# sacs-epfl/decentralized-learning-simulator

Hardware: AMD Instinct MI355X
Metric: device-resident GB/s, N-way weighted model-tensor reduce; 1/2/4/8 MI355X (higher is better)
Workload: dtype f32

## Files before the change

decentralized-learning-simulator_amd/csrc/dispatch.hpp:

```cpp
#pragma once

#include <hip/hip_runtime.h>

#include <algorithm>
#include <cmath>
#include <cstdint>
#include <cstdlib>
#include <cstring>
#include <type_traits>
#include <vector>

#include "dlsim.h"
#include "wreduce_kernels.hpp"
#include "chunk_mean_kernels.hpp"
#include "ab_env.hpp"


namespace dlsim_host __attribute__((visibility("hidden"))) {

int fail(int code, const char* fmt, ...) __attribute__((format(printf, 2, 3)));
int hip_fail(hipError_t e, const char* what);

constexpr int kVpt = 4;
constexpr size_t kBatchSmallBytes = size_t{1} << 20;
// ... 10 lines not shown
constexpr size_t kMaxLaunchOutBytes = (size_t{1} << 31) - (size_t{1} << 20);
template <class Op> constexpr int max_fixed_fan_in() { return Op::kBytes >= 4 ? 14 : 9; }
template <class Op> constexpr int group_size() { return Op::kBytes >= 4 ? 8 : 4; }

struct Shape {
  int vpt;
  int store;
  bool wave;
};
template <class Op, int C> constexpr Shape fixed_shape() {
  if constexpr (Op::kBytes >= 4) {
    if constexpr (C == 0) return Shape{2, kStore, false};
    else if constexpr (C == 1) return Shape{4, kStore, false};
    else return Shape{4, kStore, true};
  } else {
    if constexpr (C < 2) return Shape{1, kStore, true};
    else return Shape{4, dlsim::kStNT, false};
  }
}
int device_cus();
inline bool v4_tiles_even(size_t nvec) {
  const double x = static_cast<double>(nvec / (static_cast<size_t>(dlsim::kBlock) * 4)) /
                   static_cast<double>(device_cus());
  return x >= 0.75 && std::ceil(x) / x <= 1.25;
}
inline bool small_shape_r04() {
  static const bool on = dlsim::ab_getenv("DLSIM_SMALL_SHAPE_R04") != nullptr;
  return on;
}
template <class Op> int size_class(size_t nelem, int fixed_fan_in = 0) {
  const size_t bytes = nelem * Op::kBytes;
  if constexpr (Op::kBytes >= 4) {
    if (bytes < 8000000)
      return Op::kBytes == 4 && fixed_fan_in >= 6 && !small_shape_r04() && v4_tiles_even(nelem / Op::E) ? 1 : 0;
    return bytes < 20000000 ? 1 : 2;
  } else {
    return bytes < 96000000 ? 0 : 2;
  }
}

inline bool aligned16(const void* p) { return (reinterpret_cast<uintptr_t>(p) & 15u) == 0; }

template <class S> inline const void* pre_ptr(const S& s, int nf, int i) { return i < nf ? s.p[i] : nullptr; }
static_assert(dlsim::kPre == 5, "the launches below pass five leading pointers");

template <class Op, class S, int NF, int VPT, int STP, bool WAVE>
hipError_t launch_shape(const S& s, int n, void* out, size_t nelem, hipStream_t st) {
  const size_t nvec = nelem / Op::E;
  const size_t tile = static_cast<size_t>(dlsim::kBlock) * VPT;
  const size_t blocks = nvec / tile + 1;
  if (blocks > 0x7fffffffu) return hipErrorInvalidValue;
  hipLaunchKernelGGL((dlsim::k_wreduce_tiles<Op, S, NF, group_size<Op>(), VPT, kNT, STP, WAVE>),
                     dim3(static_cast<unsigned>(blocks)), dim3(dlsim::kBlock), 0, st, s, n, out, nvec, nelem);
  return hipGetLastError();
}

template <class Op, int C> constexpr Shape grouped_shape() {
  if constexpr (C == 0) return Shape{1, kStore, true};
  else if constexpr (Op::kBytes >= 4) return Shape{4, kStore, false};
  else return Shape{4, dlsim::kStNT, false};
}

template <class Op, class S, int NF, int C>
hipError_t launch_class(const S& s, int n, void* out, size_t nelem, hipStream_t st) {
  constexpr Shape k = NF > 0 ? fixed_shape<Op, C>() : grouped_shape<Op, C>();
  return launch_shape<Op, S, NF, k.vpt, k.store, k.wave>(s, n, out, nelem, st);
}

constexpr int kDeferU = 2, kDeferRMin = 4, kDeferOneRoundMax = 24;
template <class Op, int NF> constexpr int defer_rmax() { return NF >= 12 ? 24 : 32; }
template <class Op, int NF> constexpr bool defer_eligible() { return Op::kBytes == 4 && (NF >= 2 || NF == 0); }
inline int defer_min_fan_in() {
  static const int k = [] {
    const char* e = dlsim::ab_getenv("DLSIM_DEFER_MIN_FAN_IN");
    return e ? std::atoi(e) : 3;
  }();
  return k;
}
constexpr int kDeferWideFanIn = 10;
constexpr size_t kDeferWideRowsPerCu = 16;
inline bool defer_on() {
  static const bool on = [] {
    const char* e = dlsim::ab_getenv("DLSIM_DEFER");
    return !(e && e[0] == '0');
  }();
  return on;
}
inline int defer_max_fan_in() {
  static const int k = [] {
    const char* e = dlsim::ab_getenv("DLSIM_DEFER_MAX_FAN_IN");
    return e ? std::atoi(e) : 1 << 30;
  }();
  return k;
}
inline int defer_r_override() {
  static const int r = [] {
    const char* e = dlsim::ab_getenv("DLSIM_DEFER_R");
    return e ? std::atoi(e) : 0;
  }();
  return r;
}
inline int defer_rows(size_t nvec, size_t cus, int rmax) {
  if (defer_r_override() > 0) return std::min(defer_r_override(), rmax);
  const size_t T = (nvec + dlsim::kDeferBlock - 1) / dlsim::kDeferBlock;
  const size_t one = ((T + cus - 1) / cus + 1) & ~size_t{1};
  if (one <= static_cast<size_t>(std::min(rmax, kDeferOneRoundMax))) return std::max(static_cast<int>(one), kDeferRMin);
  const size_t two = ((T + 2 * cus - 1) / (2 * cus) + 1) & ~size_t{1};
  if (two <= static_cast<size_t>(rmax)) return static_cast<int>(two);
  int best = rmax;
  double best_cost = 1e300;
  for (int R = rmax / 2; R <= rmax; R += 2) {
    const double w = static_cast<double>((T + R - 1) / R) / static_cast<double>(cus);
    const double full = std::floor(w), x = w - full;
    const double cost = R * (full + (x > 0 ? std::max(x, 0.38 + 0.45 * x) : 0.0)) + 0.1 * std::ceil(w);
    if (cost < best_cost - 1e-9) {
      best_cost = cost;
      best = R;
    }
  }
  return best;
}

inline bool defer_grouped_on() {
  static const bool on = [] {
    const char* e = dlsim::ab_getenv("DLSIM_DEFER_GROUPED");
    return !(e && e[0] == '0');
  }();
  return on;
}
constexpr double kDeferMinMB = 10.0;
inline double defer_min_mb() {
  static const double x = [] {
    const char* e = dlsim::ab_getenv("DLSIM_DEFER_MIN_MB");
    return e ? std::atof(e) : kDeferMinMB;
  }();
  return x;
}
template <class Op> bool use_defer(int n, size_t nelem) {
  if (Op::kBytes != 4 || n < std::max(2, defer_min_fan_in()) || n > defer_max_fan_in() || !defer_on()) return false;
  if (static_cast<double>(nelem * Op::kBytes) < defer_min_mb() * 1e6) return false;
  if (n > max_fixed_fan_in<Op>()) return defer_grouped_on();
  if (n <= kDeferWideFanIn) return true;
  const size_t rows = nelem / Op::E / dlsim::kDeferBlock;
  return rows >= kDeferWideRowsPerCu * static_cast<size_t>(device_cus());
}

template <class Op> const char* kernel_name(int n, size_t nelem) {
  if (nelem == 0 || n < 1) return "";
  const size_t first = std::min(nelem, kMaxLaunchOutBytes / Op::kBytes);
  if (use_defer<Op>(n, first)) return n <= max_fixed_fan_in<Op>() ? "dlsim::k_wreduce_defer_pre" : "dlsim::k_wreduce_defer";
  return "dlsim::k_wreduce_tiles";
}

template <class Op, class S, int NF, int RC>
hipError_t launch_defer_kernel(const S& s, int n, void* out, size_t nvec, size_t nelem, int R, unsigned blocks,
                               hipStream_t st) {
  if constexpr (NF > 0) {
    hipLaunchKernelGGL(
        (dlsim::k_wreduce_defer_pre<Op, S, NF, group_size<Op>(), defer_rmax<Op, NF>(), kDeferU, kStore, RC>),
        dim3(blocks), dim3(dlsim::kDeferBlock), 0, st, nvec, out, pre_ptr(s, NF, 0), pre_ptr(s, NF, 1),
        pre_ptr(s, NF, 2), pre_ptr(s, NF, 3), pre_ptr(s, NF, 4), s, n, R, nelem);
  } else {
    hipLaunchKernelGGL(
        (dlsim::k_wreduce_defer<Op, S, NF, group_size<Op>(), defer_rmax<Op, NF>(), kDeferU, kStore, RC>),
        dim3(blocks), dim3(dlsim::kDeferBlock), 0, st, s, n, R, out, nvec, nelem);
  }
  return hipGetLastError();
}

template <class Op, class S, int NF, int RC>
hipError_t launch_defer_rc(const S& s, int n, void* out, size_t nvec, size_t nelem, int R, unsigned blocks,
                           hipStream_t st) {
  if constexpr (RC > defer_rmax<Op, NF>()) {
    return launch_defer_kernel<Op, S, NF, 0>(s, n, out, nvec, nelem, R, blocks, st);
  } else {
    if (R == RC) return launch_defer_kernel<Op, S, NF, RC>(s, n, out, nvec, nelem, R, blocks, st);
    return launch_defer_rc<Op, S, NF, RC + kDeferU>(s, n, out, nvec, nelem, R, blocks, st);
  }
}

template <class Op, class S, int NF>
hipError_t launch_defer(const S& s, int n, void* out, size_t nelem, hipStream_t st) {
  const size_t nvec = nelem / Op::E;
  const int R = defer_rows(nvec, static_cast<size_t>(device_cus()), defer_rmax<Op, NF>());
  const size_t span = static_cast<size_t>(dlsim::kDeferBlock) * static_cast<size_t>(R);
  const size_t blocks = (nvec + span - 1) / span;
  if (blocks == 0 || blocks > 0x7fffffffu) return hipErrorInvalidValue;
  if constexpr (NF >= 3 && std::is_same<Op, dlsim::F32Exact>::value)
    return launch_defer_rc<Op, S, NF, kDeferRMin>(s, n, out, nvec, nelem, R, static_cast<unsigned>(blocks), st);
  return launch_defer_kernel<Op, S, NF, 0>(s, n, out, nvec, nelem, R, static_cast<unsigned>(blocks), st);
}

template <class Op, class S, int NF>
hipError_t launch_tiles(const S& s, int n, void* out, size_t nelem, hipStream_t st) {
  if constexpr (NF > 0) {
    const int c = size_class<Op>(nelem, NF);
    if constexpr (defer_eligible<Op, NF>())
      if (use_defer<Op>(NF, nelem)) return launch_defer<Op, S, NF>(s, n, out, nelem, st);
    switch (c) {
      case 0: return launch_class<Op, S, NF, 0>(s, n, out, nelem, st);
      case 1: return launch_class<Op, S, NF, 1>(s, n, out, nelem, st);
      default: return launch_class<Op, S, NF, 2>(s, n, out, nelem, st);
    }
  } else {
    if constexpr (defer_eligible<Op, 0>())
      if (use_defer<Op>(n, nelem)) return launch_defer<Op, S, 0>(s, n, out, nelem, st);
    return size_class<Op>(nelem) == 0 ? launch_class<Op, S, 0, 0>(s, n, out, nelem, st)
                                      : launch_class<Op, S, 0, 2>(s, n, out, nelem, st);
  }
}

template <class Op, int K>
hipError_t launch_fixed_k(const dlsim::Slots<16, dlsim::wt_t<Op>>& s, int n, void* out, size_t nelem,
                          hipStream_t st) {
  if constexpr (K > max_fixed_fan_in<Op>()) {
    return hipErrorInvalidValue;
  } else {
    if (n == K) return launch_tiles<Op, dlsim::Slots<16, dlsim::wt_t<Op>>, K>(s, n, out, nelem, st);
    return launch_fixed_k<Op, K + 1>(s, n, out, nelem, st);
  }
}

template <class Op, class S>
hipError_t launch_any(const S& s, int n, void* out, size_t nelem, bool vec, hipStream_t st) {
  if (vec) {
    if constexpr (std::is_same<S, dlsim::Slots<16, dlsim::wt_t<Op>>>::value) {
      if (n <= max_fixed_fan_in<Op>()) return launch_fixed_k<Op, 1>(s, n, out, nelem, st);
    }
    return launch_tiles<Op, S, 0>(s, n, out, nelem, st);
  }
  const size_t blocks = (nelem + dlsim::kBlock - 1) / dlsim::kBlock;
  if (blocks > 0x7fffffffu) return hipErrorInvalidValue;
  hipLaunchKernelGGL((dlsim::k_wreduce_scalar<Op, S>), dim3(static_cast<unsigned>(blocks)), dim3(dlsim::kBlock), 0,
                     st, s, n, out, nelem);
  return hipGetLastError();
}

template <int NB, class W>
void fill_slots(dlsim::Slots<NB, W>& s, const void* const* in, const W* w, int n, float div) {
  std::memset(&s, 0, sizeof(s));
  for (int i = 0; i < n; ++i) {
    s.p[i] = in[i];
    s.w[i] = w ? w[i] : 1.0f;
  }
  s.div = div;
}

template <class Op>
int run_range(const void* const* in, int n, const dlsim::wt_t<Op>* w, void* out, size_t nelem, bool vec, float div,
              hipStream_t st) {
  using W = dlsim::wt_t<Op>;
  hipError_t e;
  if (n <= 16) {
    dlsim::Slots<16, W> s;
    fill_slots(s, in, w, n, div);
    e = launch_any<Op>(s, n, out, nelem, vec, st);
  } else if (n <= DLSIM_MAX_FUSED_INPUTS) {
    dlsim::Slots<DLSIM_MAX_FUSED_INPUTS, W> s;
    fill_slots(s, in, w, n, div);
    e = launch_any<Op>(s, n, out, nelem, vec, st);
  } else {
    const size_t pbytes = static_cast<size_t>(n) * sizeof(void*);
    std::vector<unsigned char> h(pbytes + static_cast<size_t>(n) * sizeof(W));
    std::memcpy(h.data(), in, pbytes);
    for (int i = 0; i < n; ++i) {
      const W wi = w ? w[i] : W(1);
      std::memcpy(h.data() + pbytes + static_cast<size_t>(i) * sizeof(W), &wi, sizeof(W));
    }
    void* d = nullptr;
    e = hipMallocAsync(&d, h.size(), st);
    if (e != hipSuccess) return hip_fail(e, "fan-in table alloc");
    e = hipMemcpyAsync(d, h.data(), h.size(), hipMemcpyHostToDevice, st);
    if (e == hipSuccess) {
      const dlsim::DevSlots<W> s{static_cast<const void* const*>(d),
                                 reinterpret_cast<const W*>(static_cast<unsigned char*>(d) + pbytes), div};
      e = launch_any<Op>(s, n, out, nelem, vec, st);
    }
    const hipError_t e2 = hipFreeAsync(d, st);
    if (e == hipSuccess) e = e2;
  }
  if (e != hipSuccess) return hip_fail(e, "kernel launch");
  return DLSIM_OK;
}

template <class Op>
int run(const void* const* in, int n, const dlsim::wt_t<Op>* w, void* out, size_t nelem, hipStream_t st,
        float div = 1.0f) {
  if (nelem == 0) return DLSIM_OK;
  bool vec = aligned16(out);
  for (int i = 0; i < n && vec; ++i) vec = aligned16(in[i]);
  const size_t chunk = kMaxLaunchOutBytes / Op::kBytes;
  if (!vec || nelem <= chunk) return run_range<Op>(in, n, w, out, nelem, vec, div, st);
  std::vector<const void*> sub(static_cast<size_t>(n));
  for (size_t b = 0; b < nelem; b += chunk) {
    const size_t len = std::min(chunk, nelem - b);
    for (int i = 0; i < n; ++i) sub[i] = static_cast<const char*>(in[i]) + b * Op::kBytes;
    int rc = run_range<Op>(sub.data(), n, w, static_cast<char*>(out) + b * Op::kBytes, len, vec, div, st);
    if (rc != DLSIM_OK) return rc;
  }
  return DLSIM_OK;
}

struct Span {
  uintptr_t a, b;
  int task;
};

inline bool cross_task_overlap(int nt, const int* fan_in, const void* const* in, void* const* outs, const size_t* nelem,
                        size_t esz) {
  std::vector<Span> wr;
  wr.reserve(static_cast<size_t>(nt));
  for (int t = 0; t < nt; ++t) {
    if (nelem[t] == 0) continue;
    const uintptr_t a = reinterpret_cast<uintptr_t>(outs[t]);
// ... 558 lines not shown
```

decentralized-learning-simulator_amd/csrc/wreduce_kernels.hpp:

```cpp
#pragma once

#include <hip/hip_runtime.h>
#include <stdint.h>

#include <type_traits>

#pragma clang fp contract(off)

namespace dlsim {

constexpr int kBlock = 256;

typedef uint32_t u32x4 __attribute__((ext_vector_type(4)));
typedef float f32x2 __attribute__((ext_vector_type(2)));
typedef __bf16 bf16x2 __attribute__((ext_vector_type(2)));

__device__ __forceinline__ float bf16_round(float f) {
  uint32_t u = __float_as_uint(f);
  if ((u & 0x7fffffffu) > 0x7f800000u) return __uint_as_float(0x7fc00000u);
  u += 0x7fffu + ((u >> 16) & 1u);
  return __uint_as_float(u & 0xffff0000u);
}

__device__ __forceinline__ void bf16_round2(float& a0, float& a1) {
// ... 203 lines not shown
  using T = double;
  using W = double;
  static constexpr int E = 2;
  static constexpr int kBytes = 8;
  static constexpr int kFmt = kFmtF32;
  __device__ static double init(double) { return 0.0; }
  __device__ static double step(double acc, double, double x) { return acc + x; }
  __device__ static void step2(double& a0, double& a1, double, double x0, double x1) {
    a0 = a0 + x0;
    a1 = a1 + x1;
  }
  __device__ static double finish(double a, float div) { return a / static_cast<double>(div); }
};

template <class Op>
__device__ __forceinline__ void unpack(const u32x4& r, acc_t<Op> (&x)[Op::E]) {
  if constexpr (Op::kBytes == 8) {
#pragma unroll
    for (int e = 0; e < 2; ++e)
      x[e] = __builtin_bit_cast(double, static_cast<uint64_t>(r[2 * e]) | (static_cast<uint64_t>(r[2 * e + 1]) << 32));
  } else if constexpr (Op::kBytes == 4) {
#pragma unroll
    for (int e = 0; e < 4; ++e) x[e] = __uint_as_float(r[e]);
  } else if constexpr (Op::kFmt == kFmtF16) {
#pragma unroll
    for (int e = 0; e < 4; ++e) {
      const uint32_t u = r[e];
      x[2 * e] = static_cast<float>(__builtin_bit_cast(_Float16, static_cast<uint16_t>(u & 0xffffu)));
      x[2 * e + 1] = static_cast<float>(__builtin_bit_cast(_Float16, static_cast<uint16_t>(u >> 16)));
    }
  } else {
#pragma unroll
    for (int e = 0; e < 4; ++e) {
      x[2 * e] = __uint_as_float(r[e] << 16);
      x[2 * e + 1] = __uint_as_float(r[e] & 0xffff0000u);
    }
  }
}

template <class Op>
__device__ __forceinline__ u32x4 pack(const acc_t<Op> (&a)[Op::E], float div) {
  u32x4 r;
  if constexpr (Op::kBytes == 8) {
#pragma unroll
    for (int e = 0; e < 2; ++e) {
      const uint64_t u = __builtin_bit_cast(uint64_t, Op::finish(a[e], div));
      r[2 * e] = static_cast<uint32_t>(u);
      r[2 * e + 1] = static_cast<uint32_t>(u >> 32);
    }
  } else if constexpr (Op::kBytes == 4) {
#pragma unroll
    for (int e = 0; e < 4; ++e) r[e] = __float_as_uint(Op::finish(a[e], div));
  } else if constexpr (Op::kFmt == kFmtF16) {
#pragma unroll
    for (int e = 0; e < 4; ++e) {
      const uint32_t lo = __builtin_bit_cast(uint16_t, static_cast<_Float16>(Op::finish(a[2 * e], div)));
      const uint32_t hi = __builtin_bit_cast(uint16_t, static_cast<_Float16>(Op::finish(a[2 * e + 1], div)));
      r[e] = lo | (hi << 16);
    }
  } else {
#pragma unroll
    for (int e = 0; e < 4; ++e) {
      const uint32_t lo = __float_as_uint(Op::finish(a[2 * e], div)) >> 16;
      const uint32_t hi = __float_as_uint(Op::finish(a[2 * e + 1], div)) & 0xffff0000u;
      r[e] = lo | hi;
    }
  }
  return r;
}

template <class Op>
__device__ __forceinline__ acc_t<Op> load_elem(const void* p, size_t j) {
  if constexpr (Op::kBytes == 8) {
    return static_cast<const double*>(p)[j];
  } else if constexpr (Op::kBytes == 4) {
    return static_cast<const float*>(p)[j];
  } else if constexpr (Op::kFmt == kFmtF16) {
    return static_cast<float>(static_cast<const _Float16*>(p)[j]);
  } else {
    return __uint_as_float(static_cast<uint32_t>(static_cast<const uint16_t*>(p)[j]) << 16);
  }
}

template <class Op>
__device__ __forceinline__ void store_elem(void* p, size_t j, acc_t<Op> a, float div) {
  if constexpr (Op::kBytes == 8) {
    static_cast<double*>(p)[j] = Op::finish(a, div);
  } else if constexpr (Op::kBytes == 4) {
    static_cast<float*>(p)[j] = Op::finish(a, div);
  } else if constexpr (Op::kFmt == kFmtF16) {
    static_cast<_Float16*>(p)[j] = static_cast<_Float16>(Op::finish(a, div));
  } else {
    static_cast<uint16_t*>(p)[j] = static_cast<uint16_t>(__float_as_uint(Op::finish(a, div)) >> 16);
  }
}

constexpr int kLdBuffer = 100;

template <int LDP>
__device__ __forceinline__ u32x4 ld16(const void* base, size_t v) {
  if constexpr (LDP >= kLdBuffer) {
    const __amdgpu_buffer_rsrc_t r =
        __builtin_amdgcn_make_buffer_rsrc(const_cast<void*>(base), 0, 0x7fffffff, 0x00020000);
    return __builtin_bit_cast(u32x4, __builtin_amdgcn_raw_buffer_load_b128(r, static_cast<int>(v * 16), 0,
                                                                           LDP - kLdBuffer));
  } else {
    const u32x4* p = static_cast<const u32x4*>(base) + v;
    if constexpr (LDP == 1) return __builtin_nontemporal_load(p);
    else return *p;
  }
}

template <bool NT>
__device__ __forceinline__ void st16(void* base, size_t v, const u32x4& r) {
  u32x4* p = static_cast<u32x4*>(base) + v;
  if constexpr (NT) __builtin_nontemporal_store(r, p);
  else *p = r;
}

constexpr int kStPlain = -1;
constexpr int kStNT = -2;

struct OutRef {
  void* ptr;
  __amdgpu_buffer_rsrc_t rsrc;
};

template <int STP>
__device__ __forceinline__ void store_vec(const OutRef& o, size_t v, const u32x4& r) {
  if constexpr (STP == kStPlain) {
    st16<false>(o.ptr, v, r);
  } else if constexpr (STP == kStNT) {
    st16<true>(o.ptr, v, r);
  } else {
    __builtin_amdgcn_raw_buffer_store_b128(r, o.rsrc, static_cast<int>(v * 16), 0, STP);
  }
}

template <int STP>
__device__ __forceinline__ OutRef make_out(void* out, size_t nvec) {
  OutRef o;
  o.ptr = out;
  if constexpr (STP >= 0) {
    o.rsrc = __builtin_amdgcn_make_buffer_rsrc(out, 0, static_cast<int>(nvec * 16), 0x00020000);
  }
  return o;
}

template <int NB, class W = float>
struct Slots {
  const void* p[NB];
  W w[NB];
  float div;
  __device__ const void* ptr(int i) const { return p[i]; }
  __device__ W wt(int i) const { return w[i]; }
  __device__ float divisor() const { return div; }
};

template <class W = float>
struct DevSlots {
  const void* const* p;
  const W* w;
  float div;
  __device__ const void* ptr(int i) const { return p[i]; }
  __device__ W wt(int i) const { return w[i]; }
  __device__ float divisor() const { return div; }
};

template <class Op, class S>
__device__ __forceinline__ void fold_scalar(const S& s, int n, void* out, size_t j) {
  acc_t<Op> a = 0;
  for (int i = 0; i < n; i += 8) {
    acc_t<Op> x[8];
#pragma unroll
    for (int g = 0; g < 8; ++g) x[g] = (i + g < n) ? load_elem<Op>(s.ptr(i + g), j) : 0.0f;
    if (i == 0) a = Op::init(x[0]);
#pragma unroll
    for (int g = 0; g < 8; ++g)
      if (i + g < n) a = Op::step(a, s.wt(i + g), x[g]);
  }
  store_elem<Op>(out, j, a, s.divisor());
}

template <class Op, class S>
__global__ __launch_bounds__(kBlock) void k_wreduce_scalar(const S s, int n, void* __restrict__ out,
                                                           size_t nelem) {
  const size_t j = static_cast<size_t>(blockIdx.x) * kBlock + threadIdx.x;
  if (j < nelem) fold_scalar<Op, S>(s, n, out, j);
}

template <class Op, int VPT, int NT, bool CHECK, int VS = kBlock>
__device__ __forceinline__ void load_tile(const void* src, size_t v0, size_t nvec,
                                          u32x4 (&r)[VPT]) {
#pragma unroll
  for (int v = 0; v < VPT; ++v) {
    const size_t idx = v0 + static_cast<size_t>(v) * VS;
    if constexpr (CHECK) {
      r[v] = u32x4{0u, 0u, 0u, 0u};
      if (idx < nvec) r[v] = ld16<NT>(src, idx);
    } else {
      r[v] = ld16<NT>(src, idx);
    }
  }
}

template <class Op, int VPT>
__device__ __forceinline__ void fold_tile(acc_t<Op> (&a)[VPT][Op::E], wt_t<Op> w, const u32x4 (&r)[VPT]) {
#pragma unroll
  for (int v = 0; v < VPT; ++v) {
    acc_t<Op> x[Op::E];
    unpack<Op>(r[v], x);
#pragma unroll
    for (int e = 0; e < Op::E; e += 2) Op::step2(a[v][e], a[v][e + 1], w, x[e], x[e + 1]);
  }
}

template <class Op, int VPT>
__device__ __forceinline__ void init_tile(acc_t<Op> (&a)[VPT][Op::E], const u32x4 (&r)[VPT], bool from_acc) {
#pragma unroll
  for (int v = 0; v < VPT; ++v) {
    acc_t<Op> x[Op::E];
    unpack<Op>(r[v], x);
#pragma unroll
    for (int e = 0; e < Op::E; ++e) a[v][e] = from_acc ? x[e] : Op::init(x[e]);
  }
}

template <class Op, class S, int NF, int G, int VPT, int NT, bool CHECK, int STP, int VS = kBlock>
__device__ __forceinline__ void reduce_tile(const S& s, int n, const OutRef& out, size_t v0, size_t nvec) {
  acc_t<Op> a[VPT][Op::E];
  if constexpr (NF > 0) {
    u32x4 r[NF][VPT];
#pragma unroll
    for (int i = 0; i < NF; ++i) load_tile<Op, VPT, NT, CHECK, VS>(s.ptr(i), v0, nvec, r[i]);
    init_tile<Op, VPT>(a, r[0], false);
#pragma unroll
    for (int i = 0; i < NF; ++i) fold_tile<Op, VPT>(a, s.wt(i), r[i]);
  } else {
    {
      u32x4 r[G][VPT];
      const int cnt = n < G ? n : G;
#pragma unroll
      for (int g = 0; g < G; ++g)
        if (g < cnt) load_tile<Op, VPT, NT, CHECK, VS>(s.ptr(g), v0, nvec, r[g]);
      init_tile<Op, VPT>(a, r[0], false);
#pragma unroll
      for (int g = 0; g < G; ++g)
        if (g < cnt) fold_tile<Op, VPT>(a, s.wt(g), r[g]);
    }
    for (int i0 = G; i0 < n; i0 += G) {
      u32x4 r[G][VPT];
      const int cnt = (n - i0) < G ? (n - i0) : G;
#pragma unroll
      for (int g = 0; g < G; ++g)
        if (g < cnt) load_tile<Op, VPT, NT, CHECK, VS>(s.ptr(i0 + g), v0, nvec, r[g]);
#pragma unroll
      for (int g = 0; g < G; ++g)
        if (g < cnt) fold_tile<Op, VPT>(a, s.wt(i0 + g), r[g]);
    }
  }
#pragma unroll
  for (int v = 0; v < VPT; ++v) {
    const size_t idx = v0 + static_cast<size_t>(v) * VS;
    if (!CHECK || idx < nvec) store_vec<STP>(out, idx, pack<Op>(a[v], s.divisor()));
  }
}

template <class Op, class S, int NF, int G, int VPT, int NT, int STP, bool WAVEMAP>
__device__ __forceinline__ void tiles_body(const S& s, int n, void* __restrict__ out, size_t nvec, size_t nelem) {
  constexpr size_t kTile = static_cast<size_t>(kBlock) * VPT;
  const size_t full = nvec / kTile;
  const OutRef o = make_out<STP>(out, nvec);
  const size_t nb = gridDim.x;
  if (blockIdx.x == 0) {
    if (full * kTile < nvec)
      reduce_tile<Op, S, NF, G, VPT, NT, true, STP>(s, n, o, full * kTile + threadIdx.x, nvec);
    const size_t j = nvec * Op::E + threadIdx.x;
    if (j < nelem) fold_scalar<Op, S>(s, n, out, j);
    if (nb > 1) return;
  }
  const size_t workers = nb > 1 ? nb - 1 : 1;
  const size_t first = nb > 1 ? blockIdx.x - 1 : 0;
  if constexpr (WAVEMAP) {
    const size_t lane_off = (threadIdx.x >> 6) * 64 * VPT + (threadIdx.x & 63);
    for (size_t t = first; t < full; t += workers)
      reduce_tile<Op, S, NF, G, VPT, NT, false, STP, 64>(s, n, o, t * kTile + lane_off, nvec);
  } else {
    for (size_t t = first; t < full; t += workers)
      reduce_tile<Op, S, NF, G, VPT, NT, false, STP>(s, n, o, t * kTile + threadIdx.x, nvec);
  }
}

template <class Op, class S, int NF, int G, int VPT, int NT, int STP = (NT ? kStNT : kStPlain),
          bool WAVEMAP = false>
__global__ __launch_bounds__(kBlock) void k_wreduce_tiles(const S s, int n, void* __restrict__ out, size_t nvec,
                                                          size_t nelem) {
  tiles_body<Op, S, NF, G, VPT, NT, STP, WAVEMAP>(s, n, out, nvec, nelem);
}

constexpr int kPre = 5;
template <class S>
struct PreSlots {
  const void* q[kPre];
  const S& s;
  __device__ const void* ptr(int i) const { return i < kPre ? q[i] : s.ptr(i); }
  __device__ auto wt(int i) const { return s.wt(i); }
  __device__ float divisor() const { return s.divisor(); }
};


constexpr int kDeferBlock = 512;
template <class Op, class S, int NF, int G, int U>
__device__ __forceinline__ void defer_fold_group(const S& s, int i0, int cnt, size_t base, int r0, int R, bool first,
                                                 acc_t<Op> (&a)[U][1][Op::E]) {
  constexpr int K = NF > 0 ? NF : G;
  u32x4 x[K][U];
#pragma unroll
  for (int g = 0; g < K; ++g)
    if (NF > 0 || g < cnt)
#pragma unroll
      for (int u = 0; u < U; ++u) {
        const int row = r0 + u < R ? r0 + u : r0;
        x[g][u] = ld16<1>(s.ptr(i0 + g), base + static_cast<size_t>(row) * kDeferBlock);
      }
#pragma unroll
  for (int u = 0; u < U; ++u) {
    if (first) {
      const u32x4 x0[1] = {x[0][u]};
      init_tile<Op, 1>(a[u], x0, false);
    }
#pragma unroll
    for (int g = 0; g < K; ++g)
      if (NF > 0 || g < cnt) {
        const u32x4 xg[1] = {x[g][u]};
        fold_tile<Op, 1>(a[u], s.wt(i0 + g), xg);
      }
  }
}
template <int NF, int RC> constexpr int defer_burst() { return RC <= 24 ? 2 : NF; }
template <class Op, class S, int NF, int G, int RC, int U, int STP>
__device__ __forceinline__ void defer_rows_c(const S& s, int n, const OutRef& o, size_t base) {
  static_assert(RC % U == 0, "whole row groups");
  u32x4 res[RC];
#pragma unroll
  for (int r0 = 0; r0 < RC; r0 += U) {
    if constexpr (NF == 0) {
      acc_t<Op> a[U][1][Op::E];
      defer_fold_group<Op, S, 0, G, U>(s, 0, n < G ? n : G, base, r0, RC, true, a);
      for (int i0 = G; i0 < n; i0 += G)
        defer_fold_group<Op, S, 0, G, U>(s, i0, (n - i0) < G ? (n - i0) : G, base, r0, RC, false, a);
#pragma unroll
      for (int u = 0; u < U; ++u) res[r0 + u] = pack<Op>(a[u][0], s.divisor());
    } else if constexpr (defer_burst<NF, RC>() < NF) {
      constexpr int K = defer_burst<NF, RC>();
      acc_t<Op> a[U][1][Op::E];
#pragma unroll
      for (int i0 = 0; i0 < NF; i0 += K) {
        u32x4 x[K][U];
#pragma unroll
        for (int g = 0; g < K; ++g)
#pragma unroll
          for (int u = 0; u < U; ++u)
            if (i0 + g < NF) x[g][u] = ld16<1>(s.ptr(i0 + g), base + static_cast<size_t>(r0 + u) * kDeferBlock);
        asm volatile("" ::: "memory");
        __builtin_amdgcn_sched_barrier(0);
#pragma unroll
        for (int u = 0; u < U; ++u) {
          if (i0 == 0) {
            const u32x4 x0[1] = {x[0][u]};
            init_tile<Op, 1>(a[u], x0, false);
          }
#pragma unroll
          for (int g = 0; g < K; ++g)
            if (i0 + g < NF) {
              const u32x4 xg[1] = {x[g][u]};
              fold_tile<Op, 1>(a[u], s.wt(i0 + g), xg);
            }
#pragma unroll
          for (int e = 0; e < Op::E; ++e) asm volatile("" : "+v"(a[u][0][e]) : : "memory");
        }
        __builtin_amdgcn_sched_barrier(0);
      }
#pragma unroll
      for (int u = 0; u < U; ++u) res[r0 + u] = pack<Op>(a[u][0], s.divisor());
    } else {
      u32x4 x[NF][U];
#pragma unroll
      for (int i = 0; i < NF; ++i)
#pragma unroll
        for (int u = 0; u < U; ++u) x[i][u] = ld16<1>(s.ptr(i), base + static_cast<size_t>(r0 + u) * kDeferBlock);
#pragma unroll
      for (int u = 0; u < U; ++u) {
        acc_t<Op> a[1][Op::E];
        const u32x4 x0[1] = {x[0][u]};
        init_tile<Op, 1>(a, x0, false);
#pragma unroll
        for (int i = 0; i < NF; ++i) {
          const u32x4 xi[1] = {x[i][u]};
          fold_tile<Op, 1>(a, s.wt(i), xi);
        }
        res[r0 + u] = pack<Op>(a[0], s.divisor());
      }
    }
    asm volatile("" ::: "memory");
    __builtin_amdgcn_sched_barrier(0);
  }
#pragma unroll
  for (int r = 0; r < RC; ++r) store_vec<STP>(o, base + static_cast<size_t>(r) * kDeferBlock, res[r]);
}
template <class Op, class S, int NF, int G, int RMAX, int U, int STP>
__device__ __forceinline__ void defer_rows(const S& s, int n, const OutRef& o, size_t base, int R, size_t nvec) {
  u32x4 res[RMAX];
#pragma unroll
  for (int r0 = 0; r0 < RMAX; r0 += U) {
    if (r0 < R) {
      if constexpr (NF > 0) {
        u32x4 x[NF][U];
#pragma unroll
        for (int i = 0; i < NF; ++i)
#pragma unroll
          for (int u = 0; u < U; ++u) {
            const int row = r0 + u < R ? r0 + u : r0;
            x[i][u] = ld16<1>(s.ptr(i), base + static_cast<size_t>(row) * kDeferBlock);
          }
#pragma unroll
        for (int u = 0; u < U; ++u) {
          acc_t<Op> a[1][Op::E];
          const u32x4 x0[1] = {x[0][u]};
          init_tile<Op, 1>(a, x0, false);
#pragma unroll
          for (int i = 0; i < NF; ++i) {
            const u32x4 xi[1] = {x[i][u]};
            fold_tile<Op, 1>(a, s.wt(i), xi);
          }
          res[r0 + u] = pack<Op>(a[0], s.divisor());
        }
      } else {
        acc_t<Op> a[U][1][Op::E];
        defer_fold_group<Op, S, 0, G, U>(s, 0, n < G ? n : G, base, r0, R, true, a);
        for (int i0 = G; i0 < n; i0 += G)
          defer_fold_group<Op, S, 0, G, U>(s, i0, (n - i0) < G ? (n - i0) : G, base, r0, R, false, a);
#pragma unroll
        for (int u = 0; u < U; ++u) res[r0 + u] = pack<Op>(a[u][0], s.divisor());
      }
    }
    asm volatile("" ::: "memory");
    __builtin_amdgcn_sched_barrier(0);
  }
  static_assert(STP >= 0, "buffer stores: out-of-range rows are dropped");
#pragma unroll
  for (int r = 0; r < RMAX; ++r)
    store_vec<STP>(o, r < R ? base + static_cast<size_t>(r) * kDeferBlock : nvec, res[r]);
}
template <class Op, class S, int NF, int G, int RMAX, int U, int STP, int RC>
__device__ __forceinline__ void defer_body(const S& s, int n, int Rrt, void* __restrict__ out, size_t nvec,
                                           size_t nelem) {
  const int R = RC > 0 ? RC : Rrt;
  const size_t span = static_cast<size_t>(kDeferBlock) * static_cast<size_t>(R);
  const size_t base = static_cast<size_t>(blockIdx.x) * span + threadIdx.x;
  const OutRef o = make_out<STP>(out, nvec);
  if (static_cast<size_t>(blockIdx.x + 1) * span <= nvec) {
    if constexpr (RC > 0 && NF > 0) {
      defer_rows_c<Op, S, NF, G, RC, U, STP>(s, n, o, base);
    } else if constexpr (RC > 0) {
      const S* ks = (const S*)__builtin_amdgcn_kernarg_segment_ptr();
      defer_rows_c<Op, S, 0, G, RC, U, STP>(*ks, n, o, base);
    } else if constexpr (NF > 0) {
      defer_rows<Op, S, NF, G, RMAX, U, STP>(s, n, o, base, R, nvec);
    } else {
      const S* ks = (const S*)__builtin_amdgcn_kernarg_segment_ptr();
      defer_rows<Op, S, NF, G, RMAX, U, STP>(*ks, n, o, base, R, nvec);
    }
  } else {
    for (int r = 0; r < R; ++r)
      reduce_tile<Op, S, NF, G, 1, 1, true, STP, kDeferBlock>(s, NF > 0 ? NF : n, o,
                                                              base + static_cast<size_t>(r) * kDeferBlock, nvec);
  }
  if (blockIdx.x == 0) {
    const size_t j = nvec * Op::E + threadIdx.x;
    if (j < nelem) fold_scalar<Op, S>(s, NF > 0 ? NF : n, out, j);
  }
}

template <class Op, class S, int NF, int G, int RMAX, int U, int STP, int RC = 0>
__global__ __launch_bounds__(kDeferBlock) void k_wreduce_defer(const S s, int n, int Rrt, void* __restrict__ out,
                                                               size_t nvec, size_t nelem) {
  defer_body<Op, S, NF, G, RMAX, U, STP, RC>(s, n, Rrt, out, nvec, nelem);
}

template <class Op, class S, int NF, int G, int RMAX, int U, int STP, int RC = 0>
__global__ __launch_bounds__(kDeferBlock) void k_wreduce_defer_pre(size_t nvec, void* __restrict__ out,
                                                                   const void* q0, const void* q1, const void* q2,
                                                                   const void* q3, const void* q4, const S s, int n,
                                                                   int Rrt, size_t nelem) {
  static_assert(NF > 0, "fixed fan-in");
  const PreSlots<S> ps{{q0, q1, q2, q3, q4}, s};
  defer_body<Op, PreSlots<S>, NF, G, RMAX, U, STP, RC>(ps, n, Rrt, out, nvec, nelem);
}

constexpr int kBatchMaxTasks = 32;
constexpr int kBatchMaxPtrs = 192;

struct BatchSlots {
  const void* p[kBatchMaxPtrs];
  float w[kBatchMaxPtrs];
  void* out[kBatchMaxTasks];
  size_t nvec[kBatchMaxTasks];
  size_t nelem[kBatchMaxTasks];
  float div[kBatchMaxTasks];
  uint32_t block_start[kBatchMaxTasks + 1];
  uint32_t ptr_off[kBatchMaxTasks];
  uint32_t fan_in[kBatchMaxTasks];
  int ntasks;
};
static_assert(sizeof(BatchSlots) <= 4096, "kernel arguments");

__device__ __forceinline__ int batch_find_task(const BatchSlots& s, uint32_t f) {
  int t = 0;
#pragma unroll
  for (int j = 1; j < kBatchMaxTasks; ++j) t += (j < s.ntasks && f >= s.block_start[j]) ? 1 : 0;
  return t;
}

struct TaskArgs {
  const BatchSlots& b;
  int off;
  float d;
  __device__ const void* ptr(int i) const { return b.p[off + i]; }
  __device__ float wt(int i) const { return b.w[off + i]; }
  __device__ float divisor() const { return d; }
};

template <class Op, int NF, int G, int VPT, int NT, int STP, bool WAVEMAP = false>
__global__ __launch_bounds__(kBlock) void k_wreduce_batch(const BatchSlots s) {
  const uint32_t bid = blockIdx.x;
  int t = 0;
  uint32_t local = 0;
  if (bid < static_cast<uint32_t>(s.ntasks)) {
    t = static_cast<int>(bid);
  } else {
    const uint32_t f = bid - static_cast<uint32_t>(s.ntasks);
    t = batch_find_task(s, f);
    local = f - s.block_start[t] + 1;
  }
  const TaskArgs a{s, static_cast<int>(s.ptr_off[t]), s.div[t]};
  const int n = NF > 0 ? NF : static_cast<int>(s.fan_in[t]);
  const size_t nvec = s.nvec[t];
  constexpr size_t kTile = static_cast<size_t>(kBlock) * VPT;
  const size_t full = nvec / kTile;
  const OutRef o = make_out<STP>(s.out[t], nvec);
  if (local == 0) {
    if (full * kTile < nvec)
      reduce_tile<Op, TaskArgs, NF, G, VPT, NT, true, STP>(a, n, o, full * kTile + threadIdx.x, nvec);
    const size_t j = nvec * Op::E + threadIdx.x;
    if (j < s.nelem[t]) fold_scalar<Op, TaskArgs>(a, n, s.out[t], j);
    return;
  }
  if constexpr (WAVEMAP) {
    const size_t lane_off = (threadIdx.x >> 6) * 64 * VPT + (threadIdx.x & 63);
    reduce_tile<Op, TaskArgs, NF, G, VPT, NT, false, STP, 64>(a, n, o, (local - 1) * kTile + lane_off, nvec);
  } else {
    reduce_tile<Op, TaskArgs, NF, G, VPT, NT, false, STP>(a, n, o, (local - 1) * kTile + threadIdx.x, nvec);
  }
}

struct BatchTableHeader {
  uint32_t ntasks;
  uint32_t nblocks;
  uint32_t uniform_fan_in;
  uint32_t vpt;
  uint64_t tasks_off;
  uint64_t map_off;
  uint64_t ptrs_off;
  uint64_t w_off;
};

struct BatchTaskDesc {
  void* out;
  uint64_t nvec;
  uint64_t nelem;
  uint32_t block_start;
  uint32_t ptr_off;
  uint32_t fan_in;
  uint32_t reserved;
};

struct TableArgs {
  const void* const* p;
  const float* w;
  __device__ const void* ptr(int i) const { return p[i]; }
  __device__ float wt(int i) const { return w[i]; }
  __device__ float divisor() const { return 1.0f; }
};

template <class Op, int NF, int G, int VPT, int NT, int STP, bool WAVEMAP = false>
__global__ __launch_bounds__(kBlock) void k_wreduce_batch_table(const unsigned char* __restrict__ table) {
  const BatchTableHeader* h = reinterpret_cast<const BatchTableHeader*>(table);
  const uint32_t* map = reinterpret_cast<const uint32_t*>(table + h->map_off);
  const uint32_t t = map[blockIdx.x];
  const BatchTaskDesc d = reinterpret_cast<const BatchTaskDesc*>(table + h->tasks_off)[t];
  const TableArgs a{reinterpret_cast<const void* const*>(table + h->ptrs_off) + d.ptr_off,
                    reinterpret_cast<const float*>(table + h->w_off) + d.ptr_off};
  const int n = NF > 0 ? NF : static_cast<int>(d.fan_in);
  const size_t nvec = d.nvec;
  constexpr size_t kTile = static_cast<size_t>(kBlock) * VPT;
  const size_t full = nvec / kTile;
  const OutRef o = make_out<STP>(d.out, nvec);
  const uint32_t local = blockIdx.x < h->ntasks ? 0u : blockIdx.x - d.block_start;
  if (local == 0) {
    if (full * kTile < nvec)
      reduce_tile<Op, TableArgs, NF, G, VPT, NT, true, STP>(a, n, o, full * kTile + threadIdx.x, nvec);
    const size_t j = nvec * Op::E + threadIdx.x;
    if (j < d.nelem) fold_scalar<Op, TableArgs>(a, n, d.out, j);
    return;
  }
  if constexpr (WAVEMAP) {
    const size_t lane_off = (threadIdx.x >> 6) * 64 * VPT + (threadIdx.x & 63);
    reduce_tile<Op, TableArgs, NF, G, VPT, NT, false, STP, 64>(a, n, o, (local - 1) * kTile + lane_off, nvec);
  } else {
    reduce_tile<Op, TableArgs, NF, G, VPT, NT, false, STP>(a, n, o, (local - 1) * kTile + threadIdx.x, nvec);
  }
}

template <int BYTES>
struct XorProbe {
  static constexpr int E = 16 / BYTES;
  static constexpr int kBytes = BYTES;
  static constexpr int kFmt = BYTES == 4 ? kFmtF32 : kFmtBF16;
  __device__ static float init(float) { return 0.0f; }
  __device__ static float step(float acc, float, float x) {
    float r = __uint_as_float(__float_as_uint(acc) ^ __float_as_uint(x));
    asm volatile("" : "+v"(r));
    return r;
  }
  __device__ static void step2(float& a0, float& a1, float w, float x0, float x1) {
    a0 = step(a0, w, x0);
    a1 = step(a1, w, x1);
  }
  __device__ static float finish(float a, float) { return a; }
};

constexpr int kMixedMaxInputs = 32;
struct MixedSlots {
  const void* p[kMixedMaxInputs];
  double w[kMixedMaxInputs];
  int dt[kMixedMaxInputs];
  int n;
  int out_dt;
  int seed;
};
// ... 64 lines not shown
```

Baseline: 6736.

## Load deferred-reduce inputs in two-input bursts and reserve dynamic LDS to cap occupancy

Adds a burst variant of the fixed fan-in deferred reduce that loads inputs two at a time across rows before folding, instead of loading all NF inputs up front. Also adds a grouped-burst path with nontemporal loads for variable fan-in padded slots. When the grid exceeds the CU count, launches reserve a large dynamic LDS allocation, which limits resident blocks per CU. The aim is to shape memory-request streams and reduce register pressure and DRAM contention. The risk is lower memory-level parallelism from the fewer loads in flight and lower occupancy.

```diff
diff --git a/decentralized-learning-simulator_amd/csrc/dispatch.hpp b/decentralized-learning-simulator_amd/csrc/dispatch.hpp
--- a/decentralized-learning-simulator_amd/csrc/dispatch.hpp
+++ b/decentralized-learning-simulator_amd/csrc/dispatch.hpp
@@ -186,14 +186,48 @@
   return "dlsim::k_wreduce_tiles";
 }
 
+constexpr int kDeferBurst = 2, kDeferBurstMaxRows = 24;
+inline bool defer_burst_on() {
+  static const bool on = [] {
+    const char* e = dlsim::ab_getenv("DLSIM_DEFER_BURST");
+    return !(e && e[0] == '0');
+  }();
+  return on;
+}
+constexpr unsigned kDeferLdsKB = 96;
+inline unsigned defer_lds_bytes() {
+  static const unsigned b = [] {
+    const char* e = dlsim::ab_getenv("DLSIM_DEFER_LDS_KB");
+    return (e ? static_cast<unsigned>(std::atoi(e)) : kDeferLdsKB) * 1024u;
+  }();
+  return b;
+}
+template <class K> hipError_t defer_launch_lds(K k, unsigned blocks, unsigned* lds) {
+  *lds = blocks > static_cast<unsigned>(device_cus()) ? defer_lds_bytes() : 0;
+  if (*lds <= 64 * 1024) return hipSuccess;
+  return hipFuncSetAttribute(reinterpret_cast<const void*>(k), hipFuncAttributeMaxDynamicSharedMemorySize,
+                             static_cast<int>(*lds));
+}
 template <class Op, class S, int NF, int RC>
 hipError_t launch_defer_kernel(const S& s, int n, void* out, size_t nvec, size_t nelem, int R, unsigned blocks,
                                hipStream_t st) {
+  if constexpr (NF > kDeferBurst && RC == 0) {
+    if (R <= kDeferBurstMaxRows && defer_burst_on()) {
+      const auto k =
+          dlsim::k_wreduce_defer_pre_b<kDeferBurst, Op, S, NF, group_size<Op>(), defer_rmax<Op, NF>(), kDeferU, kStore>;
+      unsigned lds = 0;
+      if (const hipError_t e = defer_launch_lds(k, blocks, &lds); e != hipSuccess) return e;
+      hipLaunchKernelGGL(k, dim3(blocks), dim3(dlsim::kDeferBlock), lds, st, nvec, out, pre_ptr(s, NF, 0),
+                         pre_ptr(s, NF, 1), pre_ptr(s, NF, 2), pre_ptr(s, NF, 3), pre_ptr(s, NF, 4), s, n, R, nelem);
+      return hipGetLastError();
+    }
+  }
   if constexpr (NF > 0) {
-    hipLaunchKernelGGL(
-        (dlsim::k_wreduce_defer_pre<Op, S, NF, group_size<Op>(), defer_rmax<Op, NF>(), kDeferU, kStore, RC>),
-        dim3(blocks), dim3(dlsim::kDeferBlock), 0, st, nvec, out, pre_ptr(s, NF, 0), pre_ptr(s, NF, 1),
-        pre_ptr(s, NF, 2), pre_ptr(s, NF, 3), pre_ptr(s, NF, 4), s, n, R, nelem);
+    const auto k = dlsim::k_wreduce_defer_pre<Op, S, NF, group_size<Op>(), defer_rmax<Op, NF>(), kDeferU, kStore, RC>;
+    unsigned lds = 0;
+    if (const hipError_t e = defer_launch_lds(k, blocks, &lds); e != hipSuccess) return e;
+    hipLaunchKernelGGL(k, dim3(blocks), dim3(dlsim::kDeferBlock), lds, st, nvec, out, pre_ptr(s, NF, 0),
+                       pre_ptr(s, NF, 1), pre_ptr(s, NF, 2), pre_ptr(s, NF, 3), pre_ptr(s, NF, 4), s, n, R, nelem);
   } else {
     hipLaunchKernelGGL(
         (dlsim::k_wreduce_defer<Op, S, NF, group_size<Op>(), defer_rmax<Op, NF>(), kDeferU, kStore, RC>),
diff --git a/decentralized-learning-simulator_amd/csrc/wreduce_kernels.hpp b/decentralized-learning-simulator_amd/csrc/wreduce_kernels.hpp
--- a/decentralized-learning-simulator_amd/csrc/wreduce_kernels.hpp
+++ b/decentralized-learning-simulator_amd/csrc/wreduce_kernels.hpp
@@ -379,6 +379,7 @@
   const void* p[NB];
   W w[NB];
   float div;
+  static constexpr bool kPadded = true;
   __device__ const void* ptr(int i) const { return p[i]; }
   __device__ W wt(int i) const { return w[i]; }
   __device__ float divisor() const { return div; }
@@ -389,6 +390,7 @@
   const void* const* p;
   const W* w;
   float div;
+  static constexpr bool kPadded = false;
   __device__ const void* ptr(int i) const { return p[i]; }
   __device__ W wt(int i) const { return w[i]; }
   __device__ float divisor() const { return div; }
@@ -635,13 +637,121 @@
 #pragma unroll
   for (int r = 0; r < RC; ++r) store_vec<STP>(o, base + static_cast<size_t>(r) * kDeferBlock, res[r]);
 }
-template <class Op, class S, int NF, int G, int RMAX, int U, int STP>
+template <class Op, class S, int G, int U, bool FULL>
+__device__ __forceinline__ void defer_burst_group(const S& s, int i0, int cnt, size_t base, int r0, int R, bool first,
+                                                  acc_t<Op> (&a)[U][1][Op::E]) {
+  static_assert(G % 2 == 0, "bursts of two inputs");
+  static_assert(S::kPadded, "reads all G slots of the remainder group");
+  typedef __attribute__((address_space(1))) const u32x4* GlobalVec;
+  GlobalVec p[G];
+  wt_t<Op> w[G];
+#pragma unroll
+  for (int g = 0; g < G; ++g) {
+    p[g] = (GlobalVec)s.ptr(i0 + g);
+    w[g] = s.wt(i0 + g);
+  }
+#pragma unroll
+  for (int g = 0; g < G; ++g) asm volatile("" : "+s"(p[g]), "+s"(w[g]));
+  size_t v[U];
+#pragma unroll
+  for (int u = 0; u < U; ++u) v[u] = base + static_cast<size_t>(r0 + u < R ? r0 + u : r0) * kDeferBlock;
+  __builtin_amdgcn_sched_barrier(0);
+#pragma unroll
+  for (int g0 = 0; g0 < G; g0 += 2) {
+    if (FULL || g0 < cnt) {
+      const bool two = FULL || g0 + 1 < cnt;
+      u32x4 x[2][U];
+#pragma unroll
+      for (int u = 0; u < U; ++u) x[0][u] = __builtin_nontemporal_load(p[g0] + v[u]);
+      if (two) {
+#pragma unroll
+        for (int u = 0; u < U; ++u) x[1][u] = __builtin_nontemporal_load(p[g0 + 1] + v[u]);
+      }
+      asm volatile("" ::: "memory");
+      __builtin_amdgcn_sched_barrier(0);
+#pragma unroll
+      for (int u = 0; u < U; ++u) {
+        if (g0 == 0 && first) {
+          const u32x4 x0[1] = {x[0][u]};
+          init_tile<Op, 1>(a[u], x0, false);
+        }
+        const u32x4 xa[1] = {x[0][u]};
+        fold_tile<Op, 1>(a[u], w[g0], xa);
+        if (two) {
+          const u32x4 xb[1] = {x[1][u]};
+          fold_tile<Op, 1>(a[u], w[g0 + 1], xb);
+        }
+#pragma unroll
+        for (int e = 0; e < Op::E; ++e) asm volatile("" : "+v"(a[u][0][e]) : : "memory");
+      }
+      __builtin_amdgcn_sched_barrier(0);
+    }
+  }
+}
+template <class Op, class S, int G, int RMAX, int U, int R0>
+__device__ __forceinline__ void defer_grouped_rows(const S& s, int n, size_t base, int R, u32x4 (&res)[RMAX]) {
+  if constexpr (R0 < RMAX) {
+    if (R0 < R) {
+      acc_t<Op> a[U][1][Op::E];
+      int i0 = 0;
+#pragma clang loop unroll(disable)
+      for (; i0 + G <= n; i0 += G) defer_burst_group<Op, S, G, U, true>(s, i0, G, base, R0, R, i0 == 0, a);
+      if (i0 < n) defer_burst_group<Op, S, G, U, false>(s, i0, n - i0, base, R0, R, i0 == 0, a);
+#pragma unroll
+      for (int u = 0; u < U; ++u) res[R0 + u] = pack<Op>(a[u][0], s.divisor());
+    }
+    asm volatile("" ::: "memory");
+    __builtin_amdgcn_sched_barrier(0);
+    defer_grouped_rows<Op, S, G, RMAX, U, R0 + U>(s, n, base, R, res);
+  }
+}
+template <class S, int NF> constexpr bool defer_group_bursts() {
+  if constexpr (NF == 0) return S::kPadded;
+  else return false;
+}
+template <class Op, class S, int NF, int G, int RMAX, int U, int STP, int KB = 0>
 __device__ __forceinline__ void defer_rows(const S& s, int n, const OutRef& o, size_t base, int R, size_t nvec) {
   u32x4 res[RMAX];
-#pragma unroll
-  for (int r0 = 0; r0 < RMAX; r0 += U) {
+  constexpr bool kGroupBursts = defer_group_bursts<S, NF>();
+  if constexpr (kGroupBursts) defer_grouped_rows<Op, S, G, RMAX, U, 0>(s, n, base, R, res);
+#pragma unroll
+  for (int r0 = 0; !kGroupBursts && r0 < RMAX; r0 += U) {
     if (r0 < R) {
-      if constexpr (NF > 0) {
+      if constexpr (NF > 0 && KB > 0 && KB < NF) {
+        size_t v[U];
+#pragma unroll
+        for (int u = 0; u < U; ++u) v[u] = base + static_cast<size_t>(r0 + u < R ? r0 + u : r0) * kDeferBlock;
+        acc_t<Op> a[U][1][Op::E];
+#pragma unroll
+        for (int i0 = 0; i0 < NF; i0 += KB) {
+          u32x4 x[KB][U];
+#pragma unroll
+          for (int g = 0; g < KB; ++g)
+#pragma unroll
+            for (int u = 0; u < U; ++u)
+              if (i0 + g < NF) x[g][u] = ld16<1>(s.ptr(i0 + g), v[u]);
+          asm volatile("" ::: "memory");
+          __builtin_amdgcn_sched_barrier(0);
+#pragma unroll
+          for (int u = 0; u < U; ++u) {
+            if (i0 == 0) {
+              const u32x4 x0[1] = {x[0][u]};
+              init_tile<Op, 1>(a[u], x0, false);
+            }
+#pragma unroll
+            for (int g = 0; g < KB; ++g)
+              if (i0 + g < NF) {
+                const u32x4 xg[1] = {x[g][u]};
+                fold_tile<Op, 1>(a[u], s.wt(i0 + g), xg);
+              }
+#pragma unroll
+            for (int e = 0; e < Op::E; ++e) asm volatile("" : "+v"(a[u][0][e]) : : "memory");
+          }
+          __builtin_amdgcn_sched_barrier(0);
+        }
+#pragma unroll
+        for (int u = 0; u < U; ++u) res[r0 + u] = pack<Op>(a[u][0], s.divisor());
+      } else if constexpr (NF > 0) {
         u32x4 x[NF][U];
 #pragma unroll
         for (int i = 0; i < NF; ++i)
@@ -679,7 +789,7 @@
   for (int r = 0; r < RMAX; ++r)
     store_vec<STP>(o, r < R ? base + static_cast<size_t>(r) * kDeferBlock : nvec, res[r]);
 }
-template <class Op, class S, int NF, int G, int RMAX, int U, int STP, int RC>
+template <class Op, class S, int NF, int G, int RMAX, int U, int STP, int RC, int KB = 0>
 __device__ __forceinline__ void defer_body(const S& s, int n, int Rrt, void* __restrict__ out, size_t nvec,
                                            size_t nelem) {
   const int R = RC > 0 ? RC : Rrt;
@@ -693,7 +803,7 @@
       const S* ks = (const S*)__builtin_amdgcn_kernarg_segment_ptr();
       defer_rows_c<Op, S, 0, G, RC, U, STP>(*ks, n, o, base);
     } else if constexpr (NF > 0) {
-      defer_rows<Op, S, NF, G, RMAX, U, STP>(s, n, o, base, R, nvec);
+      defer_rows<Op, S, NF, G, RMAX, U, STP, KB>(s, n, o, base, R, nvec);
     } else {
       const S* ks = (const S*)__builtin_amdgcn_kernarg_segment_ptr();
       defer_rows<Op, S, NF, G, RMAX, U, STP>(*ks, n, o, base, R, nvec);
@@ -723,6 +833,16 @@
   static_assert(NF > 0, "fixed fan-in");
   const PreSlots<S> ps{{q0, q1, q2, q3, q4}, s};
   defer_body<Op, PreSlots<S>, NF, G, RMAX, U, STP, RC>(ps, n, Rrt, out, nvec, nelem);
+}
+
+template <int KB, class Op, class S, int NF, int G, int RMAX, int U, int STP>
+__global__ __launch_bounds__(kDeferBlock) void k_wreduce_defer_pre_b(size_t nvec, void* __restrict__ out,
+                                                                     const void* q0, const void* q1, const void* q2,
+                                                                     const void* q3, const void* q4, const S s, int n,
+                                                                     int Rrt, size_t nelem) {
+  static_assert(NF > KB && KB > 0, "fixed fan-in of more than one burst");
+  const PreSlots<S> ps{{q0, q1, q2, q3, q4}, s};
+  defer_body<Op, PreSlots<S>, NF, G, RMAX, U, STP, 0, KB>(ps, n, Rrt, out, nvec, nelem);
 }
 
 constexpr int kBatchMaxTasks = 32;
```

Measured after the change: 6741, median of 5. Within noise of the previous version (+0.1%).
